# hyperplane-lab/RGBManip

Hardware: AMD Instinct MI355X
Metric: adapose_poses_per_sec_batch256 (higher is better)
Workload: dtype bf16

## Files before the change

### rgbmanip_amd/csrc/kernels.h

```cpp
#pragma once
#include <vector>

#include "common.h"

namespace rgbm {

int launch_nchw_to_nhwc_pad(int dtype, const float* in, void* out, int V, int C, int H, int W, int Cp, hipStream_t s);
int launch_maxpool3x3s2(int dtype, const void* in, void* out, int V, int H, int W, int C, hipStream_t s);
int launch_resize_bilinear_ac(int dtype, const void* in, void* out, int V, int Hs, int Ws, int C, int Ho, int Wo, int ldo,
                              int ch_off, hipStream_t s);
int launch_copy_channels(int dtype, const void* in, void* out, long long npix, int C, int ldo, int ch_off, hipStream_t s);
int launch_adaptive_avgpool(int dtype, const void* in, void* out, int V, int H, int W, int C, int S, hipStream_t s);
int launch_adaptive_avgpool_multi(int dtype, const void* in, void* const* outs, const int* bins, int nb, int V, int H, int W, int C,
                                  hipStream_t s);
int launch_psp_pool_conv(int dtype, const void* in, int ldi, const void* const* w, void* const* outs, const int* bins, int V, int H, int W,
                         int act, float slope, hipStream_t s);
int launch_psp_resize_cat(int dtype, const void* f, const void* const* stages, const int* bins, void* out, int V, int Ho, int Wo, hipStream_t s);
int launch_homography(const float* P_views, float* out, int V, int B, hipStream_t s);
int launch_build_volume(int dtype, const void* feat, const float* homog, const float* depths, void* vol, int v0, int Vc, int V,
                        int B, int D, int H, int W, hipStream_t s);

int launch_upconv_combine(int dtype, const void* z, const float* bias, void* out, int V, int h, int w, int Co, int ldo, int act,
                          float slope, hipStream_t s, const float* drop = nullptr);
int launch_upconv_final(int dtype, const void* x, const void* wz, const float* bias, float slope, const void* wf, const float* biasf,
                        void* out, int out_f32, int V, int h, int w, hipStream_t s, const void* wf_f16 = nullptr);

constexpr int kDropoutPerView = 256 + 64;
unsigned dropout_threshold(float p);
float dropout_scale(float p);
int launch_dropout_masks(float* masks, unsigned long long* state, int B, float p, unsigned long long seed, int advance, hipStream_t s);

size_t bn_scratch_bytes(int V);
int launch_bn_per_sample(int dtype, void* y, const void* res, const float* gamma, const float* beta, void* scratch, int V,
                         long long nvox, int C, int relu, hipStream_t s);

int launch_to_f32(int dtype, const void* in, float* out, long long n, hipStream_t s);

int launch_gather_points(int dtype, const void* feat, const int* choose, float* out, int V, int P, int HW, int C, hipStream_t s);
int launch_prob_softmax_depth(int dtype, const void* u11, const float* wprob, const int* choose, const float* depths,
                              float* prob, float* depth_out, int v0, int Vc, int B, int P, int D, int H, int W, int classmajor,
                              hipStream_t s);
int launch_dense_depth(int dtype, const void* u11, const float* wprob, const float* depths, float* depth_map, float* conf_map,
                       int v0, int Vc, int B, int D, int H, int W, int classmajor, hipStream_t s);
int launch_depth_to_points(const float* depth, const double* Kc, const double* E, int n, int S, float* points, hipStream_t s);
int launch_depth_consistency(const float* depth_a, const float* conf_a, const unsigned char* mask_a, const double* Ka, const double* Ea,
                             const float* depth_b, const double* Kb, const double* Eb, int n, int S, double px_max, double rel_max,
                             float conf_min, float* fused, float* reproj, float* rel, unsigned char* keep, hipStream_t s);
int launch_cloud_pack(const float* fused1, const unsigned char* keep1, const double* K1, const double* E1, const float* fused2,
                      const unsigned char* keep2, const double* K2, const double* E2, int n, int S, int cap, float* cloud, int* index,
                      int* count, hipStream_t s);
int launch_fuse_points(int dtype, const void* feat, const float* homog, const float* depths, const int* choose,
                       const float* prob, float* out, int V, int B, int P, int D, int H, int W, int ldo, int ch_off,
                       hipStream_t s, int Vn = -1);
int launch_mean_points(int dtype, const void* in, float* out, float* scratch, int V, int P, int C, hipStream_t s);
int launch_f32_to_f16(const float* in, void* out, long long n, hipStream_t s);
void stem_pack(const float* w, std::vector<float>& packed);
int launch_stem(int dtype, const float* img1, const float* img2, const void* wpk, void* out, int B, int V, int S, hipStream_t s);
int launch_stem_views(int dtype, const float* img, const void* wpk, void* out, int V, int S, hipStream_t s);
int launch_feature_store(const void* src, void* pool, const int* slots, int V, int pool_records, size_t part_off, size_t part_bytes,
                         size_t record_bytes, hipStream_t s);
int launch_feature_gather(const void* pool, void* dst, const int* slot1, const int* slot2, int B, int pool_records, size_t part_off,
                          size_t part_bytes, size_t record_bytes, hipStream_t s);
int launch_feature_bad_slot_nan(const int* slot1, const int* slot2, int B, int pool_records, float* const out[10], const int per_pose[10],
                                hipStream_t s);
int launch_crop_fingerprint(const float* img, int V, int n_words, unsigned long long* keys_out, hipStream_t s);
int launch_f32_to_bx3(const float* in, void* out, long long n, hipStream_t s);
int launch_view_linear(const float* x, const float* W, const float* bias, float* out, int V, int I, int O, int ldw, int i0,
                       int relu, hipStream_t s);
struct PointMlpDesc {
  const float* table;
  const void* feat;
  const int* choose;
  float* nocs4;
  float* pf;
  int ldpf, P, HW;
  long long N;
};
int point_mlp_table_floats();
void point_mlp_pack(const float* const w[6], const float* const b[6], float* table);
int launch_point_mlp(int feat_dtype, const PointMlpDesc& d, hipStream_t s);
int launch_dense_nocs(int feat_dtype, const float* table, const void* feat, float* out, long long N, hipStream_t s);
int launch_ortho6d(const float* r6, float* R, int V, hipStream_t s);
int launch_mean_points_partial(int dtype, const void* in, float* scratch, int V, int P, int C, hipStream_t s);
int launch_view_linear_mean(const float* partial, int P, float* mean_out, const float* W, const float* bias, float* out, int V, int I, int O,
                            int ldw, int i0, int relu, hipStream_t s);
int launch_pose_heads_mean(const float* partial, int P, float* mean_out, float* R, float* const w[3][3], float* const b[3][3],
                           float* const out[3], const int odim[3], int V, hipStream_t s);
constexpr int kMeanSplit = 8;
constexpr int kPoseMlpSlab = 128;
struct PoseMlpDesc {
  const float* pf96;
  const void* w[4];
  int ldw[4];
  const float* bias[4];
  const float* vbias;
  void* q128;
  float* part128;
  float* part256;
  int V, P;
};
bool pose_mlp_fits(int P);
int launch_pose_mlp1(const PoseMlpDesc& d, hipStream_t s);
int launch_pose_mlp2(const PoseMlpDesc& d, hipStream_t s);
int launch_pose_heads(const float* pf2, float* const w[3][3], float* const b[3][3], float* const out[3], const int odim[3], int V,
                      hipStream_t s);
int launch_stage_in(const float* P1, const float* P2, const int* c1, const int* c2, float* Pviews, int* choose, int B, int P, hipStream_t s);
int launch_stage_out(const float* nocs4, const float* depth, const float* R, const float* tv, const float* sv, float* const nocs[2],
                     float* const dep[2], float* const r[2], float* const t[2], float* const sz[2], int B, int P, int view2, hipStream_t s);
int launch_copy_cols(const float* in, float* out, long long rows, int ldi, int ldo, int n, hipStream_t s);

struct Conv3dTileDesc {
  const void* in; const void* wgt; void* out; const float* bias; const void* res;
  int N, Di, Hi, Wi;
  int Do, Ho, Wo;
  int Dq, Hq, Wq;
  int ntd, nth, ntw;
  int Cout, relu;
  const void* feat; const float* homog; const float* depths; int v0, V, B;
  int prof_variant; double algo_flops, algo_bytes;
  int out_classmajor;
  int feat_f16;
  const int* tile_list; const int* tile_count;
  int tile_mask_stride;
  const unsigned char* tile_mask;
};
enum DebugFlag {
  DBG_NO_WS = 8, DBG_NONUNIFORM_TAPS = 16, DBG_V3_FOR_WS = 64, DBG_NO_WS64 = 128, DBG_NO_ROWHALO = 256, DBG_GENERIC_RESIZE = 512,
  DBG_PSP_STAGE_R5 = 1024, DBG_POINT_MLP_R5 = 2048, DBG_TILE_CONV0 = 4096, DBG_NO_KSPLIT = 16384, DBG_L2_SLIM_TILE = 32768,
  DBG_WS_128x256 = 65536, DBG_NO_SLIM64 = 262144, DBG_KORDER_TAPS_OUTER = 1 << 20, DBG_SWEEP_ALT_BLEND = 1 << 21, DBG_SWEEP_DOT2 = 1 << 22,
  DBG_PP_ONE_KERNEL = 1 << 23, DBG_NO_SLIM_SMALL = 1 << 24, DBG_PP_GENERIC_SELECT = 1 << 25, DBG_PP_GUARD = 1 << 26, DBG_GLOBAL_ADDR = 1 << 27,
  DBG_SWEEP_PER_TILE = 1 << 28, DBG_SPARSE_TAIL_R5 = 1 << 29, DBG_M32_TAILS_R5 = 1 << 30, DBG_POSE_MLP_R6 = 1 << 19,
};
extern int g_debug_flags;
extern long long g_ws_min_rows;
extern int g_tuning_version;
extern int g_gemm_kernel;
void conv3d_tile_pack(const float* w, const float* scale, int Cin, int Cout, int coutp, bool transposed, int dtype,
                      std::vector<float>& packed);
int launch_conv3d_tile(int layer, int dtype, const Conv3dTileDesc& d, hipStream_t s);
int sparse_mask_bytes_per_view(int S);
int sparse_mask_offset(int S, int layer);
int launch_sparse_masks(const int* choose, int v0, int Vc, int P, int S, unsigned char* masks, int* sweep_list, int* sweep_count,
                        hipStream_t s);
int conv3d_tile_dims(int layer, int dtype, int* TD, int* TH, int* TW);

void conv0_sweep_pack(const float* w, const float* scale, std::vector<float>& packed);
int launch_conv0_sweep(const Conv3dTileDesc& d, int dtype, hipStream_t s);

int conv0_sweep_x3_upload(const std::vector<float>& packed, void** dev);
int launch_conv0_sweep_x3(const Conv3dTileDesc& d, hipStream_t s);
int launch_bx3_to_f32(const void* in, float* out, long long n, hipStream_t s);

int launch_prob_sparse(const void* u9, const void* c0, const void* w11_packed, const float* bias11, const float* wprob,
                       const int* choose, const float* depths, float* prob, float* depth_out, int v0, int Vc, int B, int P,
                       int D, int H, int W, int dtype, hipStream_t s, const void* w11_taps = nullptr);
void prob_sparse_pack(const float* w, const float* scale, std::vector<float>& packed);

int launch_prepare_inputs(const float* rgb, const unsigned char* mask, const double* K, const int* frame_map, int N, int H, int W, int S, int P,
                          unsigned seed, float* img, int* choose, float* pts2d, double* Kcrop, int* window, int* valid,
                          unsigned char* small_scratch, hipStream_t s, int frame0 = 0);
int launch_prepare_inputs_u8(const unsigned char* rgb, const unsigned char* mask, const double* K, const int* frame_map, int N, int H, int W,
                             int S, int P, unsigned seed, float* img, int* choose, float* pts2d, double* Kcrop, int* window, int* valid,
                             unsigned char* small_scratch, hipStream_t s, int frame0 = 0);
int launch_prepare_inputs_opt(const void* rgb, int pixel_type, int normalize, const unsigned char* mask, const double* K, const int* frame_map,
                              int N, int H, int W, int S, int P, unsigned seed, float* img, int* choose, float* pts2d, double* Kcrop,
                              int* window, int* valid, unsigned char* small_scratch, hipStream_t s, int frame0 = 0);
int launch_prepare_inputs_windows(const void* pix, int pixel_type, int normalize, const unsigned char* mask_pix, const long long* offset,
                                  const int* window, const int* valid_in, const double* K, int frame0, int N, int H, int W, int S, int P,
                                  unsigned seed, float* img, int* choose, float* pts2d, double* Kcrop, int* valid, unsigned char* small_scratch,
                                  hipStream_t s);
int launch_quantize_frames(const float* src, unsigned char* dst, size_t n, hipStream_t s);

int launch_umeyama_ransac(const float* nocs, const float* depth, const int* choose, const double* Kc, const double* E1,
                          double* bbox, double* srt, int* valid, int B, int P, int img, unsigned seed, hipStream_t s);

int launch_cloud_gather(const float* map1, const float* map2, const int* index, int n, int S2, int C, int cap, float* out, hipStream_t s);
size_t cloud_similarity_scratch_bytes(int n, int cap);
int launch_cloud_similarity(const float* nocs, const float* cloud, const int* count, int n, int cap, unsigned seed, double* bbox, double* srt,
                            int* info, int* valid, void* scratch, size_t scratch_bytes, hipStream_t s);

int launch_projection(const double* Kc, const double* E, float* P, int n, hipStream_t s);
int launch_pnp_ransac(const float* nocs1, const float* pts1, const float* nocs2, const float* pts2, const double* K, const double* E1,
                      const double* E2, double* bbox, double* srt, int* info, int* valid, int B, int P, unsigned seed, hipStream_t s);

int launch_mask_extent(const unsigned char* mask, int N, int H, int W, int* ext, int* count, hipStream_t s);

int launch_postprocess(const float* nocs, const float* depth, const float* rot, const int* choose, const double* Kc,
                       const double* E1, double* bbox, double* ts_out, int* valid, int B, int P, int img, hipStream_t s,
                       void* scratch = nullptr, size_t scratch_bytes = 0);
int launch_postprocess_regressed(const float* nocs, const float* rot, const float* tr, const float* sv, const double* E1, double* bbox,
                                 double* ts_out, int* valid, int B, int P, hipStream_t s);
int launch_microbench_mfma(float* scratch, int iters, int random_operands, double* flops, hipStream_t s);
int microbench_mfma_scratch_floats(int* n);
int launch_microbench_copy(const void* src, void* dst, size_t bytes, hipStream_t s);
size_t postprocess_scratch_bytes(int B);
int postprocess_slices(int B);

int launch_gae(int T, int N, const float* rewards, const unsigned char* dones, const float* values, const float* last_values,
               float gamma, float lam, float* returns, float* adv, double* sums, hipStream_t s);
int launch_adv_normalise(long long n_local, float* adv, const double* sums, double count_total, hipStream_t s);

struct PolicyLayout { int dims[5]; int log_std; int w[2][4]; int b[2][4]; int total; };
struct PolicyOptState { int t; int n_updates; float lr; float last_kl; float last_norm; float pad_; double sum_surr; double sum_vloss; };
int launch_policy_forward(const float* params, const PolicyLayout& L, int n, int mode, const float* obs, const float* noise,
                          float* actions, float* logp, float* value, float* mu, hipStream_t s);
int policy_partial_floats(const PolicyLayout& L, int n);
int launch_ppo_minibatch(const float* params, const PolicyLayout& L, int n, const float* obs, const float* actions,
                         const float* old_logp, const float* adv, const float* returns, const float* old_values,
                         const float* old_mu, const float* old_sigma, float clip, float vcoef, float ecoef, float* partial,
                         float* grads, hipStream_t s);
constexpr int POLICY_MAX_HIDDEN = 6, POLICY_MAX_WIDTH = 512, POLICY_MAX_ACT = 32;
enum { PACT_ELU = 0, PACT_SELU = 1, PACT_RELU = 2, PACT_LRELU = 3, PACT_TANH = 4, PACT_SIGMOID = 5 };
struct PolicyDesc {
  int obs_dim, state_dim, act_dim, activation, asymmetric;
  int n_hidden[2];
  int hidden[2][POLICY_MAX_HIDDEN];
  int w[2][POLICY_MAX_HIDDEN + 1];
  int b[2][POLICY_MAX_HIDDEN + 1];
  int log_std, total;
};
int launch_policy_forward_ex(const float* params, const PolicyDesc& D, int n, int mode, const float* obs, const float* states,
                             const float* noise, float* actions, float* logp, float* value, float* mu, hipStream_t s);
int ppo_scratch_floats_ex(const PolicyDesc& D, int n, int clipped_vloss, size_t* count);
int launch_ppo_minibatch_ex(const float* params, const PolicyDesc& D, int n, const float* obs, const float* states,
                            const float* actions, const float* old_logp, const float* adv, const float* returns,
                            const float* old_values, const float* old_mu, const float* old_sigma, float clip, float vcoef, float ecoef,
                            int clipped_vloss, float* scratch, float* grads, hipStream_t s);
int launch_ppo_adam(float* params, const float* grads, float* m, float* v, PolicyOptState* st, int total, float inv_world,
                    float max_norm, float desired_kl, float lr_min, float lr_max, int adaptive, hipStream_t s);

}
```

### rgbmanip_amd/csrc/upconv.hip

```cpp
#include <type_traits>

#include "common.h"
#include "kernels.h"
#include "prof.h"

namespace rgbm {

namespace {

template <typename T> struct Raw4 { typedef uint4 type; };
template <> struct Raw4<unsigned short> { typedef uint2 type; };
template <> struct Raw4<f16_t> { typedef uint2 type; };
__device__ __forceinline__ void unpack4(const uint2& r, float* v, unsigned short) {
  v[0] = __uint_as_float(r.x << 16); v[1] = __uint_as_float(r.x & 0xffff0000u);
  v[2] = __uint_as_float(r.y << 16); v[3] = __uint_as_float(r.y & 0xffff0000u);
}
__device__ __forceinline__ void unpack4(const uint2& r, float* v, f16_t) {
  const f16x4 hh = __builtin_bit_cast(f16x4, r);
#pragma unroll
  for (int e = 0; e < 4; ++e) v[e] = (float)hh[e];
}
__device__ __forceinline__ void unpack4(const uint4& r, float* v, float) { unpack_chunk(r, v, float()); }
__device__ __forceinline__ void unpack4(const uint4& r, float* v, bx3_t) { bx3_join4(r, v); }

template <typename T, int BR, int BC, int KH, int KW>
struct UpTap {
  static constexpr int E = 4;
  typedef typename Raw4<T>::type raw_t;
  static constexpr int NR = BR / 2 + 2, NC = BC / 2 + 2;
  static constexpr int JMIN = KH >> 1, JMAX = ((KH + BR - 1) >> 1) + 1;
  static constexpr int CMIN = KW >> 1, CMAX = ((KW + BC - 1) >> 1) + 1;
  __device__ static __forceinline__ void load(const T* zb, int Co, long long ldz, const int (&roff)[NR], const int (&coff)[NC],
                                              raw_t (&raw)[NR][NC]) {
    const T* zt = zb + (KH * 3 + KW) * Co;
#pragma unroll
    for (int j = JMIN; j <= JMAX; ++j)
#pragma unroll
      for (int c = CMIN; c <= CMAX; ++c) raw[j][c] = *reinterpret_cast<const raw_t*>(zt + (long long)(roff[j] + coff[c]) * ldz);
  }
  __device__ static __forceinline__ void accumulate(const raw_t (&raw)[NR][NC], const float (&wy)[BR + 2][2],
                                                    const float (&wx)[BC + 2][2], float (&acc)[BR][BC][E]) {
#pragma unroll
    for (int j = JMIN; j <= JMAX; ++j) {
      float hx[BC][E];
#pragma unroll
      for (int b = 0; b < BC; ++b) {
        const int c0 = (b + KW) >> 1;
        float p0[E], p1[E];
        unpack4(raw[j][c0], p0, T());
        unpack4(raw[j][c0 + 1], p1, T());
#pragma unroll
        for (int e = 0; e < E; ++e) hx[b][e] = fmaf(wx[b + KW][0], p0[e], wx[b + KW][1] * p1[e]);
      }
#pragma unroll
      for (int a = 0; a < BR; ++a) {
        const int ra = (a + KH) >> 1;
        if (j != ra && j != ra + 1) continue;
        const float coef = wy[a + KH][j == ra ? 0 : 1];
#pragma unroll
        for (int b = 0; b < BC; ++b)
#pragma unroll
          for (int e = 0; e < E; ++e) acc[a][b][e] = fmaf(coef, hx[b][e], acc[a][b][e]);
      }
#pragma unroll
      for (int a = 0; a < BR; ++a)
#pragma unroll
        for (int b = 0; b < BC; ++b)
          asm volatile("" : "+v"(acc[a][b][0]), "+v"(acc[a][b][1]), "+v"(acc[a][b][2]), "+v"(acc[a][b][3]));
      __builtin_amdgcn_sched_barrier(0);
    }
  }
};

template <typename T, int BR, int BC, bool DROP>
__global__ __launch_bounds__(256) __attribute__((amdgpu_waves_per_eu(sizeof(T) == 2 ? 3 : 2, 8))) void upconv_combine_kernel(const T* __restrict__ z, const float* __restrict__ bias,
                                                               T* __restrict__ out, int V, int h, int w, int Co, int ldo,
                                                               float nslope, float sy, float sx, const float* __restrict__ drop) {
  constexpr int E = 4;
  typedef typename Raw4<T>::type raw_t;
  constexpr int NR = BR / 2 + 2, NC = BC / 2 + 2;
  const int cpp = Co / E, Ho = 2 * h, Wo = 2 * w;
  const int nbi = (Ho + BR - 1) / BR, nbj = (Wo + BC - 1) / BC;
  const long long total = (long long)V * nbi * nbj * cpp;
  const long long ldz = 9ll * Co;
  const long long nchunk = (total + 255) / 256, per_xcd = (nchunk + 7) / 8;
  for (long long q = blockIdx.x; q < per_xcd * 8; q += gridDim.x) {
    const long long chunk = (q & 7) * per_xcd + (q >> 3);
    const long long idx = chunk * 256 + threadIdx.x;
    if (chunk >= nchunk || idx >= total) continue;
    const unsigned u0 = (unsigned)idx;
    const unsigned pp = u0 / (unsigned)cpp;
    const int cc = (int)(u0 - pp * (unsigned)cpp);
    const unsigned rowb = pp / (unsigned)nbj;
    const int bj = (int)(pp - rowb * (unsigned)nbj);
    const unsigned vv = rowb / (unsigned)nbi;
    const int bi = (int)(rowb - vv * (unsigned)nbi);
    const int rbase = (BR / 2) * bi - 1, cbase = (BC / 2) * bj - 1;
    float wy[BR + 2][2], wx[BC + 2][2];
#pragma unroll
    for (int k = 0; k < BR + 2; ++k) {
      const int u = BR * bi - 1 + k;
      const float rel = __fsub_rn(__fmul_rn(sy, (float)u), (float)(rbase + (k >> 1)));
      const bool ok = u >= 0 && u < Ho;
      wy[k][1] = ok ? rel : 0.f;
      wy[k][0] = ok ? 1.f - rel : 0.f;
    }
#pragma unroll
    for (int k = 0; k < BC + 2; ++k) {
      const int u = BC * bj - 1 + k;
      const float rel = __fsub_rn(__fmul_rn(sx, (float)u), (float)(cbase + (k >> 1)));
      const bool ok = u >= 0 && u < Wo;
      wx[k][1] = ok ? rel : 0.f;
      wx[k][0] = ok ? 1.f - rel : 0.f;
    }
    int roff[NR], coff[NC];
#pragma unroll
    for (int j = 0; j < NR; ++j) roff[j] = min(max(rbase + j, 0), h - 1) * w;
#pragma unroll
    for (int j = 0; j < NC; ++j) coff[j] = min(max(cbase + j, 0), w - 1);
    const T* zb = z + ((long long)vv * h * w) * ldz + cc * E;

    float acc[BR][BC][E];
    {
      float bv[E];
#pragma unroll
      for (int e = 0; e < E; ++e) bv[e] = bias ? bias[cc * E + e] : 0.f;
#pragma unroll
      for (int a = 0; a < BR; ++a)
#pragma unroll
        for (int b = 0; b < BC; ++b)
#pragma unroll
          for (int e = 0; e < E; ++e) acc[a][b][e] = bv[e];
    }
    raw_t ra[NR][NC], rb[NR][NC];
#define UP_STEP(KH0, KW0, KH1, KW1, CUR, NXT)                                        \
    UpTap<T, BR, BC, KH1, KW1>::load(zb, Co, ldz, roff, coff, NXT);                 \
    __builtin_amdgcn_sched_barrier(0);                                               \
    UpTap<T, BR, BC, KH0, KW0>::accumulate(CUR, wy, wx, acc);                        \
    __builtin_amdgcn_sched_barrier(0);
    UpTap<T, BR, BC, 0, 0>::load(zb, Co, ldz, roff, coff, ra);
    UP_STEP(0, 0, 0, 1, ra, rb)
    UP_STEP(0, 1, 0, 2, rb, ra)
    UP_STEP(0, 2, 1, 0, ra, rb)
    UP_STEP(1, 0, 1, 1, rb, ra)
    UP_STEP(1, 1, 1, 2, ra, rb)
    UP_STEP(1, 2, 2, 0, rb, ra)
    UP_STEP(2, 0, 2, 1, ra, rb)
    UP_STEP(2, 1, 2, 2, rb, ra)
#undef UP_STEP
    UpTap<T, BR, BC, 2, 2>::accumulate(ra, wy, wx, acc);
    T* ob = out + ((long long)vv * Ho * Wo) * ldo + cc * E;
    float df[E];
    if constexpr (DROP) {
      const float4 d4 = *reinterpret_cast<const float4*>(drop + (long long)vv * kDropoutPerView + cc * E);
      df[0] = d4.x; df[1] = d4.y; df[2] = d4.z; df[3] = d4.w;
    }
#pragma unroll
    for (int a = 0; a < BR; ++a) {
      const int oy = BR * bi + a;
#pragma unroll
      for (int b = 0; b < BC; ++b) {
        const int ox = BC * bj + b;
        float r[E];
#pragma unroll
        for (int e = 0; e < E; ++e) r[e] = acc[a][b][e] < 0.f ? __builtin_fmaxf(acc[a][b][e], -3.402823466e38f) * nslope : acc[a][b][e];
        if constexpr (DROP) {
#pragma unroll
          for (int e = 0; e < E; ++e) r[e] *= df[e];
        }
        store4(ob + ((long long)oy * Wo + ox) * ldo, r);
      }
    }
  }
}

template <typename T>
int launch_t(const void* z, const float* bias, void* out, int V, int h, int w, int Co, int ldo, float nslope, float sy, float sx,
             hipStream_t s, const float* drop) {
#ifndef UPC_BC
#define UPC_BC 4
#endif
  constexpr int BR = 2, BC = UPC_BC, E = 4;
  const long long total = (long long)V * ((2 * h + BR - 1) / BR) * ((2 * w + BC - 1) / BC) * (Co / E);
  RGBM_REQUIRE(total > 0 && total < (1ll << 31), "upconv combine grid out of range");
  RGBM_REQUIRE((2 * h) % BR == 0 && (2 * w) % BC == 0, "upconv combine: output size must be a multiple of the thread block shape");
  const long long blocks = (total + 255) / 256;
  const unsigned grid = (unsigned)(blocks < (1ll << 20) ? blocks : (1ll << 20));
  if (drop)
    hipLaunchKernelGGL((upconv_combine_kernel<T, BR, BC, true>), dim3(grid), dim3(256), 0, s, (const T*)z, bias, (T*)out, V, h, w, Co, ldo,
                       nslope, sy, sx, drop);
  else
    hipLaunchKernelGGL((upconv_combine_kernel<T, BR, BC, false>), dim3(grid), dim3(256), 0, s, (const T*)z, bias, (T*)out, V, h, w, Co, ldo,
                       nslope, sy, sx, drop);
  RGBM_CHECK_HIP(hipGetLastError());
  return 0;
}

}

int launch_upconv_combine(int dtype, const void* z, const float* bias, void* out, int V, int h, int w, int Co, int ldo, int act,
                          float slope, hipStream_t s, const float* drop) {
  RGBM_REQUIRE(drop == nullptr || (((uintptr_t)drop & 15) == 0 && Co <= 256), "upconv combine: dropout factors (16-byte aligned, <= 256 channels)");
  RGBM_REQUIRE(Co % 4 == 0 && ldo % dtype_chunk(dtype) == 0 && h >= 2 && w >= 2, "upconv combine geometry");
  RGBM_REQUIRE(act == ACT_NONE || act == ACT_RELU || act == ACT_PRELU, "upconv combine activation");
  const float sy = (float)(h - 1) / (float)(2 * h - 1), sx = (float)(w - 1) / (float)(2 * w - 1);
  const double nout = (double)V * 4.0 * h * w * Co;
  prof_begin_launch(s, dtype_size(dtype) == 2 ? 37 : 38, 72.0 * nout, ((double)V * h * w * 9.0 * Co + nout) * (double)dtype_size(dtype));
  const float nslope = act == ACT_NONE ? 1.f : act == ACT_RELU ? 0.f : slope;
  int rc;
  if (dtype == BF16) rc = launch_t<unsigned short>(z, bias, out, V, h, w, Co, ldo, nslope, sy, sx, s, drop);
  else if (dtype == F16) rc = launch_t<f16_t>(z, bias, out, V, h, w, Co, ldo, nslope, sy, sx, s, drop);
  else if (dtype == BF16X3) rc = launch_t<bx3_t>(z, bias, out, V, h, w, Co, ldo, nslope, sy, sx, s, drop);
  else rc = launch_t<float>(z, bias, out, V, h, w, Co, ldo, nslope, sy, sx, s, drop);
  prof_end_launch(s);
  return rc;
}

}
```

Before: 6006.

## Restructure upconv combine as row-wise separable blend with 4x4 output blocks

Replaces the per-tap pipeline in the upconv combine kernel with a row-wise scheme. For each input row it loads all three kernel-column taps, blends them horizontally once, then adds the result into every output row that uses it. This removes repeated horizontal interpolation work per tap and row pair. For 2-byte types with even input sizes, each thread now computes 4x4 outputs, so more input is reused per thread at the cost of more registers and fewer waves. The old per-tap path stays behind a debug flag, and the geometry check is relaxed to allow sizes of 1.

Result: no change. 6047 (median of 6 runs) (+0.7%).

```diff
diff --git a/rgbmanip_amd/csrc/kernels.h b/rgbmanip_amd/csrc/kernels.h
--- a/rgbmanip_amd/csrc/kernels.h
+++ b/rgbmanip_amd/csrc/kernels.h
@@ -130,6 +130,7 @@
   DBG_WS_128x256 = 65536, DBG_NO_SLIM64 = 262144, DBG_KORDER_TAPS_OUTER = 1 << 20, DBG_SWEEP_ALT_BLEND = 1 << 21, DBG_SWEEP_DOT2 = 1 << 22,
   DBG_PP_ONE_KERNEL = 1 << 23, DBG_NO_SLIM_SMALL = 1 << 24, DBG_PP_GENERIC_SELECT = 1 << 25, DBG_PP_GUARD = 1 << 26, DBG_GLOBAL_ADDR = 1 << 27,
   DBG_SWEEP_PER_TILE = 1 << 28, DBG_SPARSE_TAIL_R5 = 1 << 29, DBG_M32_TAILS_R5 = 1 << 30, DBG_POSE_MLP_R6 = 1 << 19,
+  DBG_UPCONV_PER_TAP = 32,
 };
 extern int g_debug_flags;
 extern long long g_ws_min_rows;
diff --git a/rgbmanip_amd/csrc/upconv.hip b/rgbmanip_amd/csrc/upconv.hip
--- a/rgbmanip_amd/csrc/upconv.hip
+++ b/rgbmanip_amd/csrc/upconv.hip
@@ -72,8 +72,58 @@
   }
 };
 
-template <typename T, int BR, int BC, bool DROP>
-__global__ __launch_bounds__(256) __attribute__((amdgpu_waves_per_eu(sizeof(T) == 2 ? 3 : 2, 8))) void upconv_combine_kernel(const T* __restrict__ z, const float* __restrict__ bias,
+template <typename T, int BR, int BC, int KH, int J>
+struct UpRow {
+  static constexpr int E = 4;
+  typedef typename Raw4<T>::type raw_t;
+  static constexpr int NC = BC / 2 + 2;
+  static_assert(J >= (KH >> 1) && J <= ((KH + BR - 1) >> 1) + 1, "row J is not touched by kernel row KH");
+  __device__ static __forceinline__ void load(const T* zb, int Co, long long ldz, int roff, const int (&coff)[NC], raw_t (&raw)[3][NC]) {
+#pragma unroll
+    for (int kw = 0; kw < 3; ++kw) {
+      const T* zt = zb + (KH * 3 + kw) * Co;
+#pragma unroll
+      for (int c = kw >> 1; c <= ((kw + BC - 1) >> 1) + 1; ++c) raw[kw][c] = *reinterpret_cast<const raw_t*>(zt + (long long)(roff + coff[c]) * ldz);
+    }
+  }
+  __device__ static __forceinline__ void accumulate(const raw_t (&raw)[3][NC], const float (&wy)[BR + 2][2], const float (&wx)[BC + 2][2],
+                                                    float (&acc)[BR][BC][E]) {
+    float sum[BC][E];
+#pragma unroll
+    for (int kw = 0; kw < 3; ++kw)
+#pragma unroll
+      for (int b = 0; b < BC; ++b) {
+        const int c0 = (b + kw) >> 1;
+        float p0[E], p1[E];
+        unpack4(raw[kw][c0], p0, T());
+        unpack4(raw[kw][c0 + 1], p1, T());
+#pragma unroll
+        for (int e = 0; e < E; ++e) {
+          if (kw == 0) sum[b][e] = fmaf(wx[b][0], p0[e], wx[b][1] * p1[e]);
+          else sum[b][e] = fmaf(wx[b + kw][1], p1[e], fmaf(wx[b + kw][0], p0[e], sum[b][e]));
+        }
+      }
+#pragma unroll
+    for (int a = 0; a < BR; ++a) {
+      const int ra = (a + KH) >> 1;
+      if (J != ra && J != ra + 1) continue;
+      const float coef = wy[a + KH][J == ra ? 0 : 1];
+#pragma unroll
+      for (int b = 0; b < BC; ++b)
+#pragma unroll
+        for (int e = 0; e < E; ++e) acc[a][b][e] = fmaf(coef, sum[b][e], acc[a][b][e]);
+    }
+#pragma unroll
+    for (int a = 0; a < BR; ++a)
+#pragma unroll
+      for (int b = 0; b < BC; ++b)
+        asm volatile("" : "+v"(acc[a][b][0]), "+v"(acc[a][b][1]), "+v"(acc[a][b][2]), "+v"(acc[a][b][3]));
+    __builtin_amdgcn_sched_barrier(0);
+  }
+};
+
+template <typename T, int BR, int BC, bool DROP, bool PER_TAP>
+__global__ __launch_bounds__(256) __attribute__((amdgpu_waves_per_eu(sizeof(T) == 2 && BR == 2 ? 3 : 2, 8))) void upconv_combine_kernel(const T* __restrict__ z, const float* __restrict__ bias,
                                                                T* __restrict__ out, int V, int h, int w, int Co, int ldo,
                                                                float nslope, float sy, float sx, const float* __restrict__ drop) {
   constexpr int E = 4;
@@ -132,23 +182,56 @@
 #pragma unroll
           for (int e = 0; e < E; ++e) acc[a][b][e] = bv[e];
     }
-    raw_t ra[NR][NC], rb[NR][NC];
+    if constexpr (PER_TAP) {
+      raw_t ra[NR][NC], rb[NR][NC];
 #define UP_STEP(KH0, KW0, KH1, KW1, CUR, NXT)                                        \
-    UpTap<T, BR, BC, KH1, KW1>::load(zb, Co, ldz, roff, coff, NXT);                 \
-    __builtin_amdgcn_sched_barrier(0);                                               \
-    UpTap<T, BR, BC, KH0, KW0>::accumulate(CUR, wy, wx, acc);                        \
-    __builtin_amdgcn_sched_barrier(0);
-    UpTap<T, BR, BC, 0, 0>::load(zb, Co, ldz, roff, coff, ra);
-    UP_STEP(0, 0, 0, 1, ra, rb)
-    UP_STEP(0, 1, 0, 2, rb, ra)
-    UP_STEP(0, 2, 1, 0, ra, rb)
-    UP_STEP(1, 0, 1, 1, rb, ra)
-    UP_STEP(1, 1, 1, 2, ra, rb)
-    UP_STEP(1, 2, 2, 0, rb, ra)
-    UP_STEP(2, 0, 2, 1, ra, rb)
-    UP_STEP(2, 1, 2, 2, rb, ra)
+      UpTap<T, BR, BC, KH1, KW1>::load(zb, Co, ldz, roff, coff, NXT);                 \
+      __builtin_amdgcn_sched_barrier(0);                                               \
+      UpTap<T, BR, BC, KH0, KW0>::accumulate(CUR, wy, wx, acc);                        \
+      __builtin_amdgcn_sched_barrier(0);
+      UpTap<T, BR, BC, 0, 0>::load(zb, Co, ldz, roff, coff, ra);
+      UP_STEP(0, 0, 0, 1, ra, rb)
+      UP_STEP(0, 1, 0, 2, rb, ra)
+      UP_STEP(0, 2, 1, 0, ra, rb)
+      UP_STEP(1, 0, 1, 1, rb, ra)
+      UP_STEP(1, 1, 1, 2, ra, rb)
+      UP_STEP(1, 2, 2, 0, rb, ra)
+      UP_STEP(2, 0, 2, 1, ra, rb)
+      UP_STEP(2, 1, 2, 2, rb, ra)
 #undef UP_STEP
-    UpTap<T, BR, BC, 2, 2>::accumulate(ra, wy, wx, acc);
+      UpTap<T, BR, BC, 2, 2>::accumulate(ra, wy, wx, acc);
+    } else {
+      static_assert(BR == 2 || BR == 4, "the row sequences below are those of two and of four output rows per thread");
+      raw_t r0[3][NC], r1[3][NC], r2[3][NC];
+#define UP_ROW(KH0, J0, KH2, J2, CUR, NXT)                                           \
+      UpRow<T, BR, BC, KH2, J2>::load(zb, Co, ldz, roff[J2], coff, NXT);             \
+      __builtin_amdgcn_sched_barrier(0);                                             \
+      UpRow<T, BR, BC, KH0, J0>::accumulate(CUR, wy, wx, acc);                       \
+      __builtin_amdgcn_sched_barrier(0);
+      UpRow<T, BR, BC, 0, 0>::load(zb, Co, ldz, roff[0], coff, r0);
+      UpRow<T, BR, BC, 0, 1>::load(zb, Co, ldz, roff[1], coff, r1);
+      if constexpr (BR == 2) {
+        UP_ROW(0, 0, 1, 0, r0, r2)
+        UP_ROW(0, 1, 1, 1, r1, r0)
+        UP_ROW(1, 0, 1, 2, r2, r1)
+        UP_ROW(1, 1, 2, 1, r0, r2)
+        UP_ROW(1, 2, 2, 2, r1, r0)
+        UpRow<T, BR, BC, 2, 1>::accumulate(r2, wy, wx, acc);
+        UpRow<T, BR, BC, 2, 2>::accumulate(r0, wy, wx, acc);
+      } else {
+        UP_ROW(0, 0, 0, 2, r0, r2)
+        UP_ROW(0, 1, 1, 0, r1, r0)
+        UP_ROW(0, 2, 1, 1, r2, r1)
+        UP_ROW(1, 0, 1, 2, r0, r2)
+        UP_ROW(1, 1, 1, 3, r1, r0)
+        UP_ROW(1, 2, 2, 1, r2, r1)
+        UP_ROW(1, 3, 2, 2, r0, r2)
+        UP_ROW(2, 1, 2, 3, r1, r0)
+        UpRow<T, BR, BC, 2, 2>::accumulate(r2, wy, wx, acc);
+        UpRow<T, BR, BC, 2, 3>::accumulate(r0, wy, wx, acc);
+      }
+#undef UP_ROW
+    }
     T* ob = out + ((long long)vv * Ho * Wo) * ldo + cc * E;
     float df[E];
     if constexpr (DROP) {
@@ -174,26 +257,38 @@
   }
 }
 
-template <typename T>
-int launch_t(const void* z, const float* bias, void* out, int V, int h, int w, int Co, int ldo, float nslope, float sy, float sx,
-             hipStream_t s, const float* drop) {
-#ifndef UPC_BC
-#define UPC_BC 4
-#endif
-  constexpr int BR = 2, BC = UPC_BC, E = 4;
+template <typename T, int BR, int BC, bool DROP, bool PER_TAP>
+int launch_block(const void* z, const float* bias, void* out, int V, int h, int w, int Co, int ldo, float nslope, float sy, float sx,
+                 hipStream_t s, const float* drop) {
+  constexpr int E = 4;
   const long long total = (long long)V * ((2 * h + BR - 1) / BR) * ((2 * w + BC - 1) / BC) * (Co / E);
   RGBM_REQUIRE(total > 0 && total < (1ll << 31), "upconv combine grid out of range");
   RGBM_REQUIRE((2 * h) % BR == 0 && (2 * w) % BC == 0, "upconv combine: output size must be a multiple of the thread block shape");
   const long long blocks = (total + 255) / 256;
   const unsigned grid = (unsigned)(blocks < (1ll << 20) ? blocks : (1ll << 20));
-  if (drop)
-    hipLaunchKernelGGL((upconv_combine_kernel<T, BR, BC, true>), dim3(grid), dim3(256), 0, s, (const T*)z, bias, (T*)out, V, h, w, Co, ldo,
-                       nslope, sy, sx, drop);
-  else
-    hipLaunchKernelGGL((upconv_combine_kernel<T, BR, BC, false>), dim3(grid), dim3(256), 0, s, (const T*)z, bias, (T*)out, V, h, w, Co, ldo,
-                       nslope, sy, sx, drop);
+  hipLaunchKernelGGL((upconv_combine_kernel<T, BR, BC, DROP, PER_TAP>), dim3(grid), dim3(256), 0, s, (const T*)z, bias, (T*)out, V, h, w, Co,
+                     ldo, nslope, sy, sx, drop);
   RGBM_CHECK_HIP(hipGetLastError());
   return 0;
+}
+
+template <typename T, bool DROP>
+int launch_d(const void* z, const float* bias, void* out, int V, int h, int w, int Co, int ldo, float nslope, float sy, float sx,
+             hipStream_t s, const float* drop) {
+  if (g_debug_flags & DBG_UPCONV_PER_TAP)
+    return w % 2 == 0 ? launch_block<T, 2, 4, DROP, true>(z, bias, out, V, h, w, Co, ldo, nslope, sy, sx, s, drop)
+                      : launch_block<T, 2, 2, DROP, true>(z, bias, out, V, h, w, Co, ldo, nslope, sy, sx, s, drop);
+  if constexpr (sizeof(T) == 2)
+    if (w % 2 == 0 && h % 2 == 0) return launch_block<T, 4, 4, DROP, false>(z, bias, out, V, h, w, Co, ldo, nslope, sy, sx, s, drop);
+  return w % 2 == 0 ? launch_block<T, 2, 4, DROP, false>(z, bias, out, V, h, w, Co, ldo, nslope, sy, sx, s, drop)
+                    : launch_block<T, 2, 2, DROP, false>(z, bias, out, V, h, w, Co, ldo, nslope, sy, sx, s, drop);
+}
+
+template <typename T>
+int launch_t(const void* z, const float* bias, void* out, int V, int h, int w, int Co, int ldo, float nslope, float sy, float sx,
+             hipStream_t s, const float* drop) {
+  return drop ? launch_d<T, true>(z, bias, out, V, h, w, Co, ldo, nslope, sy, sx, s, drop)
+              : launch_d<T, false>(z, bias, out, V, h, w, Co, ldo, nslope, sy, sx, s, drop);
 }
 
 }
@@ -201,7 +296,7 @@
 int launch_upconv_combine(int dtype, const void* z, const float* bias, void* out, int V, int h, int w, int Co, int ldo, int act,
                           float slope, hipStream_t s, const float* drop) {
   RGBM_REQUIRE(drop == nullptr || (((uintptr_t)drop & 15) == 0 && Co <= 256), "upconv combine: dropout factors (16-byte aligned, <= 256 channels)");
-  RGBM_REQUIRE(Co % 4 == 0 && ldo % dtype_chunk(dtype) == 0 && h >= 2 && w >= 2, "upconv combine geometry");
+  RGBM_REQUIRE(Co % 4 == 0 && ldo % dtype_chunk(dtype) == 0 && h >= 1 && w >= 1, "upconv combine geometry");
   RGBM_REQUIRE(act == ACT_NONE || act == ACT_RELU || act == ACT_PRELU, "upconv combine activation");
   const float sy = (float)(h - 1) / (float)(2 * h - 1), sx = (float)(w - 1) / (float)(2 * w - 1);
   const double nout = (double)V * 4.0 * h * w * Co;
```
